# HamidGadirov/OpticalFlowSciVis

Hardware: AMD Instinct MI355X
Metric: volume-pairs/sec, Flow-3D unsupervised train step (fwd+loss+bwd+AdamW) (higher is better)
Workload: dtype f32

## Files before the change

include/flowsci_hip.h:

```cpp
#ifndef FLOWSCI_HIP_H
#define FLOWSCI_HIP_H

#ifdef __cplusplus
extern "C" {
#endif

typedef void* fs_stream_t;

enum {
  FS_OK = 0,
  FS_ERR_NULLPTR = 1,
  FS_ERR_SHAPE = 2,
  FS_ERR_ARG = 3,
  FS_ERR_LAUNCH = 4,
  FS_ERR_UNSUPPORTED = 5
};

#define FS_ABI_VERSION 380
int fs_version(void);
const char* fs_error_string(int code);

int fs_warp3d_fwd(const float* in, const float* flow, float* out,
                  int B, int C, const int* in_dhw, int D, int H, int W, fs_stream_t stream);
int fs_warp3d_bwd(const float* in, const float* flow, const float* grad_out,
                  float* grad_in, float* grad_flow,
                  int B, int C, const int* in_dhw, int D, int H, int W, fs_stream_t stream);

int fs_warp3d_pair_fwd(const float* img0, const float* img1, const float* flow6,
                       float* out0, float* out1,
                       int B, int C, const int* in_dhw, int D, int H, int W, fs_stream_t stream);
int fs_warp3d_pair_bwd(const float* img0, const float* img1, const float* flow6,
                       const float* grad_out0, const float* grad_out1,
                       float* grad_img0, float* grad_img1, float* grad_flow6,
                       int B, int C, const int* in_dhw, int D, int H, int W, fs_stream_t stream);
int fs_warp3d_pair_bwd_acc(const float* img0, const float* img1, const float* flow6,
                           const float* grad_out0, const float* grad_out1,
                           float* grad_img0, float* grad_img1,
                           const float* grad_flow_add, float* grad_flow6,
                           int B, int C, const int* in_dhw, int D, int H, int W, fs_stream_t stream);

int fs_upsample_warp3d_pair_fwd(const float* img0, const float* img1, const float* delta,
                                const float* prev_flow, float* flow_out, float* out0, float* out1,
                                int B, int C, const int* in_dhw, int Ds, int Hs, int Ws, int factor,
                                float scale, fs_stream_t stream);
int fs_upsample_warp3d_pair_bwd(const float* img0, const float* img1, const float* flow6,
                                const float* grad_out0, const float* grad_out1,
                                const float* grad_flow_add, float* grad_flow_total, float* grad_delta,
                                float* ws, int B, int C, const int* in_dhw, int Ds, int Hs, int Ws,
                                int factor, float scale, fs_stream_t stream);
int fs_warp3d_pair_bwd_acc3(const float* img0, const float* img1, const float* flow6,
                            const float* grad_out0, long long gout_batch_stride0, const float* grad_out1,
                            long long gout_batch_stride1, float* grad_img0, float* grad_img1,
                            const float* add0, long long batch_stride0, const float* add1, long long batch_stride1,
                            const float* add2, long long batch_stride2, float* grad_flow6,
                            int B, int C, const int* in_dhw, int D, int H, int W, fs_stream_t stream);
int fs_upsample_warp3d_pair_bwd3(const float* img0, const float* img1, const float* flow6,
                                 const float* grad_out0, long long gout_batch_stride0, const float* grad_out1,
                                 long long gout_batch_stride1, const float* add0, long long batch_stride0, const float* add1, long long batch_stride1,
                                 const float* add2, long long batch_stride2, float* grad_flow_total, float* grad_delta,
                                 float* ws, int B, int C, const int* in_dhw, int Ds, int Hs, int Ws,
                                 int factor, float scale, fs_stream_t stream);

enum { FS_W3_KERNEL_GATHER = 0, FS_W3_KERNEL_RC = 1 };
int fs_warp3d_kernel_id(const float* in0, const float* in1, const float* flow, int B, int C, const int* in_dhw,
                        int D, int H, int W, int backward, int with_grad_in);

enum { FS_WARP2D_RIFE = 0, FS_WARP2D_PWC = 1, FS_WARP2D_PHOTO = 2, FS_WARP2D_DILATED = 3 };

int fs_warp2d_fwd(const float* in, const float* flow, const float* start, float* out,
                  int B, int C, const int* in_hw, int H, int W, int mode, int with_mask,
                  fs_stream_t stream);
int fs_warp2d_bwd(const float* in, const float* flow, const float* start,
                  const float* grad_out, float* grad_in, float* grad_flow,
                  int B, int C, const int* in_hw, int H, int W, int mode, int with_mask,
                  fs_stream_t stream);

int fs_warp2d_pair_fwd(const float* img0, const float* img1, const float* flow4,
                       float* out0, float* out1,
// ... 265 lines not shown
```

opticalflowscivis_amd/_lib.py:

```python
import ctypes
import os

import torch

_HERE = os.path.dirname(os.path.abspath(__file__))
PRODUCT_LIB_PATH = os.path.join(_HERE, "csrc", "libflowsci_hip.so")
LIB_PATH = os.environ.get("FLOWSCI_HIP_LIBRARY") or PRODUCT_LIB_PATH
ABLATION = LIB_PATH != PRODUCT_LIB_PATH


def ablation_env(name):
    return os.environ.get(name) if ABLATION else None


def switches():
    return {"library": "ablation build: " + LIB_PATH if ABLATION else "product",
            "env": {k: v for k, v in sorted(os.environ.items()) if k.startswith("FLOWSCI_")}}

ABI_VERSION = 380

_f32p = ctypes.c_void_p
_int = ctypes.c_int
_float = ctypes.c_float
_stream = ctypes.c_void_p
_intp = ctypes.POINTER(ctypes.c_int)
_i64p = ctypes.POINTER(ctypes.c_longlong)
_i64 = ctypes.c_longlong
_ptrv = ctypes.POINTER(ctypes.c_void_p)
_double = ctypes.c_double

class FsWprepJob(ctypes.Structure):
    _fields_ = [("w", ctypes.c_void_p), ("ws", ctypes.c_void_p), ("kind", ctypes.c_int), ("total", ctypes.c_int),
                ("p", ctypes.c_int * 6)]


_jobp = ctypes.POINTER(FsWprepJob)

SIGNATURES = {
    "fs_version": [],
    "fs_error_string": [_int],
    "fs_warp3d_fwd": [_f32p] * 3 + [_int, _int, _intp, _int, _int, _int, _stream],
    "fs_warp3d_bwd": [_f32p] * 5 + [_int, _int, _intp, _int, _int, _int, _stream],
    "fs_warp3d_pair_fwd": [_f32p] * 5 + [_int, _int, _intp, _int, _int, _int, _stream],
    "fs_warp3d_pair_bwd": [_f32p] * 8 + [_int, _int, _intp, _int, _int, _int, _stream],
    "fs_warp3d_pair_bwd_acc": [_f32p] * 9 + [_int, _int, _intp, _int, _int, _int, _stream],
    "fs_warp3d_pair_bwd_acc3": [_f32p] * 3 + [_f32p, _i64, _f32p, _i64] + [_f32p] * 2 + [_f32p, _i64, _f32p, _i64, _f32p, _i64, _f32p, _int, _int, _intp, _int, _int,
                                _int, _stream],
    "fs_upsample_warp3d_pair_bwd3": [_f32p] * 3 + [_f32p, _i64, _f32p, _i64] + [_f32p, _i64, _f32p, _i64, _f32p, _i64] + [_f32p] * 3 +
                                    [_int, _int, _intp, _int, _int, _int, _int, _float, _stream],
    "fs_upsample_warp3d_pair_fwd": [_f32p] * 7 + [_int, _int, _intp, _int, _int, _int, _int, _float, _stream],
    "fs_upsample_warp3d_pair_bwd": [_f32p] * 9 + [_int, _int, _intp, _int, _int, _int, _int, _float, _stream],
    "fs_warp2d_pair_fwd": [_f32p] * 5 + [_int, _int, _intp, _int, _int, _int, _stream],
    "fs_warp2d_pair_bwd": [_f32p] * 8 + [_int, _int, _intp, _int, _int, _int, _stream],
    "fs_interp3d_bwd_scaled": [_f32p] * 3 + [_int] * 10 + [_float, _stream],
    "fs_downsample3d_fwd": [_f32p] * 2 + [_int] * 6 + [_float, _stream],
    "fs_downsample3d_fwd_ms": [_ptrv, _i64p, _f32p] + [_int] * 6 + [_float, _stream],
    "fs_resize2d_fwd": [_f32p] * 2 + [_int] * 8 + [_float, _stream],
    "fs_resize2d_bwd": [_f32p] * 2 + [_int] * 8 + [_float, _stream],
    "fs_occ_check2d": [_f32p] * 4 + [_int] * 3 + [_float, _float, _int, _stream],
    "fs_laploss2d_sizes": [_int] * 4 + [_i64p] * 3,
    "fs_laploss2d_fwd": [_f32p] * 5 + [_int] * 4 + [_stream],
    "fs_laploss2d_bwd": [_f32p] * 4 + [_int] * 4 + [_stream],
    "fs_laploss3d_sizes": [_int] * 5 + [_i64p] * 3,
    "fs_laploss3d_fwd": [_f32p] * 5 + [_int] * 5 + [_stream],
    "fs_laploss3d_bwd": [_f32p] * 4 + [_int] * 5 + [_stream],
    "fs_conv3d_fwd_ws_floats": [_int] * 3,
    "fs_conv3d_fwd": [_f32p] * 5 + [_int] * 13 + [_stream],
    "fs_upsample3d_scale_add": [_f32p] * 3 + [_int] * 6 + [_float, _stream],
    "fs_conv3d_fwd_dprelu_part_floats": [_int] * 5,
    "fs_conv3d_fwd_dprelu_part_floats_k3": [_int] * 5,
# ... 44 lines not shown
    "fs_warp2d_bwd": [_f32p, _f32p, _f32p, _f32p, _f32p, _f32p, _int, _int, _intp, _int, _int, _int, _int,
                      _stream],
    "fs_frame_metrics2d_ws_bytes": [_int] * 4,
    "fs_frame_metrics3d_ws_bytes": [_int] * 5,
    "fs_frame_metrics2d": [_f32p] * 2 + [_int] * 4 + [_double] + [_f32p] * 3 + [_stream],
    "fs_frame_metrics3d": [_f32p] * 2 + [_int] * 5 + [_double] + [_f32p] * 3 + [_stream],
    "fs_flow_metrics2d_ws_bytes": [_int] * 4,
    "fs_flow_metrics3d_ws_bytes": [_int] * 6,
    "fs_flow_metrics2d": [_f32p] * 2 + [_int] * 4 + [_i64] * 2 + [_f32p] * 2 + [_float] * 2 + [_f32p] * 3 + [_stream],
    "fs_flow_metrics3d": [_f32p] * 2 + [_int] * 5 + [_i64] * 2 + [_f32p] * 2 + [_int] + [_float] * 2 + [_f32p] * 3 +
                         [_stream],
    "fs_flow_consistency2d_ws_bytes": [_int] * 4,
    "fs_flow_consistency3d_ws_bytes": [_int] * 5,
    "fs_flow_consistency2d": [_f32p] * 2 + [_int] * 4 + [_i64] * 2 + [_f32p] * 3 + [_double] * 2 + [_f32p] * 4 + [_stream],
    "fs_flow_consistency3d": [_f32p] * 2 + [_int] * 5 + [_i64] * 2 + [_f32p] * 3 + [_double] * 2 + [_f32p] * 4 + [_stream],
    "fs_triplet_gather": [_f32p, _int, _i64, _int, _int, _int, _f32p, _int, _int, _int, _int, _f32p, _stream],
    "fs_series_stats_ws_bytes": [_int, _i64],
    "fs_series_stats": [_f32p, _int, _int, _i64, _f32p, _f32p, _stream],
    "fs_census3d_dist_fwd": [_f32p] * 3 + [_int] * 5 + [_stream],
    "fs_census3d_dist_bwd": [_f32p] * 5 + [_int] * 5 + [_stream],
    "fs_flow_smooth3d_fwd": [_f32p] * 4 + [_int] * 5 + [_float] * 3 + [_stream],
    "fs_flow_smooth3d_bwd": [_f32p] * 4 + [_int] * 5 + [_float] * 3 + [_stream],
}
_RESTYPES = {"fs_error_string": ctypes.c_char_p, "fs_conv3d_fwd_ws_floats": ctypes.c_longlong,
             "fs_conv3d_wrw_det_ws_floats": ctypes.c_longlong,
             "fs_frame_metrics2d_ws_bytes": ctypes.c_longlong, "fs_frame_metrics3d_ws_bytes": ctypes.c_longlong,
             "fs_flow_metrics2d_ws_bytes": ctypes.c_longlong, "fs_flow_metrics3d_ws_bytes": ctypes.c_longlong,
             "fs_flow_consistency2d_ws_bytes": ctypes.c_longlong, "fs_flow_consistency3d_ws_bytes": ctypes.c_longlong,
             "fs_series_stats_ws_bytes": ctypes.c_longlong,
             "fs_conv3d_tr_ws_floats": ctypes.c_longlong, "fs_conv3d_fwd_dprelu_part_floats": ctypes.c_longlong,
             "fs_conv3d_fwd_dprelu_part_floats_k3": ctypes.c_longlong}


class FlowsciLibraryError(RuntimeError):
    pass


class FlowsciKernelError(RuntimeError):
    pass


_lib = None


def lib():
    global _lib
    if _lib is not None:
# ... 29 lines not shown
```

opticalflowscivis_amd/convgrad.py:

```python
import os

import torch
import torch.nn as nn
import torch.nn.functional as F


def _tuple(v, nd):
    return tuple(v) if isinstance(v, (tuple, list)) else (v,) * nd


_stock_seen = set()


def _note_stock_path(what, x, w, stride, padding):
    if x.dim() != 5 or not x.is_cuda or x.dtype != torch.float32:
        return
    key = (what, tuple(x.shape[1:]), tuple(w.shape), tuple(stride), tuple(padding))
    if key in _stock_seen:
        return
    _stock_seen.add(key)
    import warnings
    warnings.warn("opticalflowscivis_amd: %s of a 3-D convolution runs on stock ATen / MIOpen kernels, not on the HIP "
                  "implicit-GEMM kernels (input %s, weight %s, stride %s, padding %s: unsupported geometry or beyond "
                  "32-bit offsets)" % (what, tuple(x.shape), tuple(w.shape), tuple(stride), tuple(padding)),
# ... 116 lines not shown


class _ConvTrAddFn(torch.autograd.Function):

    @staticmethod
    def forward(ctx, x, w, b, addend, stride, padding):
        from . import ops
        y = ops.conv3d_tr(x, w, b, None, None, addend)
        ctx.save_for_backward(x, w)
        ctx.cfg = (stride, padding, b is not None)
        return y

    @staticmethod
    def backward(ctx, gy):
        x, w = ctx.saved_tensors
        stride, padding, has_bias = ctx.cfg
        gy = gy.contiguous()
        gx = gw = gb = None
        if ctx.needs_input_grad[0]:
            gx = _conv_grad_input(x, w, gy, stride, padding, True)
        if ctx.needs_input_grad[1]:
            gw = _conv_grad_weight(x, w, gy, stride, padding, True)
        if has_bias and ctx.needs_input_grad[2]:
            gb = gy.sum(dim=(0, 2, 3, 4))
        return gx, gw, gb, (gy if ctx.needs_input_grad[3] else None), None, None


class _ConvPReLUFn(torch.autograd.Function):

    @staticmethod
    def forward(ctx, x, w, b, a, stride, padding, transposed):
        y, z = _conv_forward(x, w, b, stride, padding, transposed, a)
        ctx.save_for_backward(x, w, y, a)
        ctx.cfg = (stride, padding, transposed, b is not None)
        return z

    @staticmethod
    def backward(ctx, gz):
        from . import ops
        x, w, y, a = ctx.saved_tensors
        stride, padding, transposed, has_bias = ctx.cfg
        gy, ga, gb = ops.prelu_backward(y, gz.contiguous(), a, want_bias_grad=has_bias)
        gx = gw = None
        if ctx.needs_input_grad[0]:
            gx = _conv_grad_input(x, w, gy, stride, padding, transposed)
        if ctx.needs_input_grad[1]:
            gw = _conv_grad_weight(x, w, gy, stride, padding, transposed)
# ... 59 lines not shown
        return None
    return _ConvPReLUCatFn.apply(conv.weight, conv.bias, act.weight, _tuple(conv.stride, 3), _tuple(conv.padding, 3),
                                 *pieces)


class _HeadFn(torch.autograd.Function):

    @staticmethod
    def forward(ctx, x, w1, b1, a1, w2, b2, addend):
        from . import ops
        y1, z1 = ops.conv3d_tr(x, w1, b1, None, a1)
        out = ops.conv3d_tr(z1, w2, b2, None, None, addend)
        ctx.save_for_backward(x, w1, a1, y1, z1, w2)
        ctx.has = (b1 is not None, b2 is not None, addend is not None)
        return out

    @staticmethod
    def backward(ctx, gout):
        from . import ops
        x, w1, a1, y1, z1, w2 = ctx.saved_tensors
        s3, p3 = (2, 2, 2), (1, 1, 1)
        gout = gout.contiguous()
        gw2 = _conv_grad_weight(z1, w2, gout, s3, p3, True) if ctx.needs_input_grad[4] else None
        gb2 = gout.sum(dim=(0, 2, 3, 4)) if (ctx.has[1] and ctx.needs_input_grad[5]) else None
        fused = ops.conv3d_deconv_grad_input_dprelu(gout, w2, y1, a1)
        if fused is not None:
            gy1, ga1, gb1 = fused
        else:
            gz1 = _conv_grad_input(z1, w2, gout, s3, p3, True)
            gy1, ga1, gb1 = ops.prelu_backward(y1, gz1, a1, want_bias_grad=ctx.has[0])
        if not ctx.has[0]:
            gb1 = None
        gw1 = _conv_grad_weight(x, w1, gy1, s3, p3, True) if ctx.needs_input_grad[1] else None
        gx = _conv_grad_input(x, w1, gy1, s3, p3, True) if ctx.needs_input_grad[0] else None
        return gx, gw1, gb1, ga1, gw2, gb2, (gout if (ctx.has[2] and ctx.needs_input_grad[6]) else None)


def head_fused_ok(head, x, addend):
    d1, act, d2 = head[0], head[1], head[2]
    if not (_hip_autograd(x) and x.dim() == 5 and x.dtype == torch.float32 and isinstance(d1, ConvTranspose3d)
            and isinstance(d2, ConvTranspose3d) and isinstance(act, nn.PReLU)):
        return False
    for d in (d1, d2):
        if not (_tuple(d.kernel_size, 3) == (4, 4, 4) and _tuple(d.stride, 3) == (2, 2, 2) and _tuple(d.padding, 3) == (1, 1, 1)
                and d.groups == 1 and _tuple(d.dilation, 3) == (1, 1, 1) and _tuple(d.output_padding, 3) == (0, 0, 0)):
            return False
    if act.weight.numel() not in (1, d1.out_channels):
# ... 130 lines not shown
```

opticalflowscivis_amd/csrc/warp3d.hip:

```cpp
#include <stdint.h>

#include <type_traits>

#include "common.hpp"

namespace {

constexpr int TH = 64;

struct W3P {
  int B, C, D, H, W;
  int Di, Hi, Wi;
  int tilesH, tilesW;
  int dc, nDC;
  float stepD, stepH, stepW;
  float rD, rH, rW;
  float mD, mH, mW;
  unsigned rowB, planeB;
  int flowC;
};

struct W3Fwd { const float* in[2]; float* out[2]; };
struct W3Bwd {
  const float* in[2]; const float* gout[2]; float* gin[2];
  long long gbs[2];
};

// ... 725 lines not shown
  if (vec && rc_mode() != 0 && rc::applicable(p, io.in[0], io.in[1]))
    return {W3K::RC, (int)FS_AB_ENV_LL("FLOWSCI_W3_RC_DC", rc::pick_dc(p, npair))};
  return {vec ? W3K::RING_VEC : W3K::RING_SCALAR, (int)FS_AB_ENV_LL("FLOWSCI_W3_RING_DC", 16)};
}

W3Pick pick_bwd(const W3P& p, const W3Bwd& io, int npair, bool with_gin, const float* flow, const float* gflow,
                const W3Add& gadd) {
  const bool vec = vec_ok(p, flow, gflow, io.gout[0], io.gout[1]) && vec_ok(p, gadd.a[0], gadd.a[1], gadd.a[2], nullptr) &&
                   gadd.bs[0] % 4 == 0 && gadd.bs[1] % 4 == 0 && gadd.bs[2] % 4 == 0 && io.gbs[0] % 4 == 0 && io.gbs[1] % 4 == 0;
  if (vec && rc_mode() != 0 && !with_gin && gflow != nullptr && rc::applicable(p, io.in[0], io.in[1]))
    return {W3K::RC, (int)FS_AB_ENV_LL("FLOWSCI_W3_RC_DC", rc::pick_dc(p, npair))};
  return {vec ? W3K::BWD_VEC : W3K::BWD_SCALAR, p.dc};
}

dim3 set_chunks(W3P& p, const W3Pick& k, int npair) {
  p.flowC = 3 * npair;
  p.dc = k.dc;
  p.nDC = fs::cdiv(p.D, p.dc);
  return dim3((unsigned)((long long)p.B * p.nDC * p.tilesH * p.tilesW), npair);
}

template <bool BWD, int NMW_, int R>
void launch_rc(const dim3& g, hipStream_t st, const W3Fwd& fio, const W3Bwd& bio, const float* flow, float* gflow,
               const W3Add& gadd, const W3P& p) {
  const dim3 bc(64 * (NCW + NMW_));
#ifdef FS_ABLATION
#define W3_RC_DBG(N) \
  if (rc_mode() == 10 + N) { hipLaunchKernelGGL((rc::warp3d_rc_kernel<BWD, NMW_, R, N>), g, bc, 0, st, fio, bio, flow, gflow, gadd, p); return; }
  W3_RC_DBG(1) W3_RC_DBG(2) W3_RC_DBG(3)
#endif
  hipLaunchKernelGGL((rc::warp3d_rc_kernel<BWD, NMW_, R>), g, bc, 0, st, fio, bio, flow, gflow, gadd, p);
}

int launch_fwd(const W3Fwd& io, int npair, const float* flow, const UpP* up, W3P& p, fs_stream_t stream) {
  const W3Pick k = pick_fwd(p, io, npair, flow, up);
  const dim3 g = set_chunks(p, k, npair);
  hipStream_t st = (hipStream_t)stream;
  switch (k.kernel) {
    case W3K::UPS_VEC: hipLaunchKernelGGL((warp3d_fwd_kernel<512, true, true>), g, dim3(512), 0, st, io, flow, *up, p); break;
    case W3K::UPS_SCALAR: hipLaunchKernelGGL((warp3d_fwd_kernel<512, false, true>), g, dim3(512), 0, st, io, flow, *up, p); break;
    case W3K::RC: launch_rc<false, 2, 6>(g, st, io, W3Bwd{}, flow, nullptr, W3Add{}, p); break;
    case W3K::RING_VEC: {
#ifdef FS_ABLATION
      static const int ring = (int)FS_AB_ENV_LL("FLOWSCI_W3_RING", 0);
#define W3_RING_CASE(R, A, DBG, ID) \
      if (ring == ID) { hipLaunchKernelGGL((warp3d_fwd_ring_kernel<true, A, R, DBG>), g, dim3(NT2), 0, st, io, flow, p); break; }
      W3_RING_CASE(3, 0, 0, 3) W3_RING_CASE(4, 0, 0, 4) W3_RING_CASE(5, 0, 0, 5) W3_RING_CASE(3, 2, 0, 13) W3_RING_CASE(5, 2, 0, 15)
      W3_RING_CASE(4, 2, 1, 101) W3_RING_CASE(4, 2, 2, 102) W3_RING_CASE(4, 2, 3, 103) W3_RING_CASE(4, 2, 4, 104) W3_RING_CASE(4, 2, 5, 105)
#endif
      hipLaunchKernelGGL((warp3d_fwd_ring_kernel<true, 2, 4>), g, dim3(NT2), 0, st, io, flow, p);
      break;
    }
    case W3K::RING_SCALAR: hipLaunchKernelGGL((warp3d_fwd_ring_kernel<false, 0, 3>), g, dim3(NT2), 0, st, io, flow, p); break;
    default: return FS_ERR_ARG;
  }
  FS_LAUNCH_CHECK();
  return FS_OK;
}

int launch_bwd(const W3Bwd& io, int npair, bool with_gin, const float* flow, float* gflow, const W3Add& gadd,
               W3P& p, fs_stream_t stream) {
  const W3Pick k = pick_bwd(p, io, npair, with_gin, flow, gflow, gadd);
  const dim3 g = set_chunks(p, k, npair);
  hipStream_t st = (hipStream_t)stream;
  switch (k.kernel) {
    case W3K::RC: launch_rc<true, 4, 5>(g, st, W3Fwd{}, io, flow, gflow, gadd, p); break;
    case W3K::BWD_VEC:
      if (with_gin) hipLaunchKernelGGL((warp3d_bwd_kernel<256, true, true>), g, dim3(256), 0, st, io, flow, gflow, gadd, p);
      else hipLaunchKernelGGL((warp3d_bwd_kernel<256, true, false>), g, dim3(256), 0, st, io, flow, gflow, gadd, p);
      break;
    case W3K::BWD_SCALAR:
      if (with_gin) hipLaunchKernelGGL((warp3d_bwd_kernel<256, false, true>), g, dim3(256), 0, st, io, flow, gflow, gadd, p);
      else hipLaunchKernelGGL((warp3d_bwd_kernel<256, false, false>), g, dim3(256), 0, st, io, flow, gflow, gadd, p);
      break;
    default: return FS_ERR_ARG;
  }
  FS_LAUNCH_CHECK();
  return FS_OK;
}

int make_params_up(W3P& p, int B, int C, const int* in_dhw, int Ds, int Hs, int Ws, int factor) {
  if (factor != 2 && factor != 4) return FS_ERR_ARG;
  if (Ds < 1 || Hs < 1 || Ws < 1) return FS_ERR_SHAPE;
  if ((long long)Ds * Hs * Ws * factor * factor * factor >= (1ll << 31)) return FS_ERR_SHAPE;
  return make_params(p, B, C, in_dhw, Ds * factor, Hs * factor, Ws * factor);
}

}

extern "C" int fs_warp3d_fwd(const float* in, const float* flow, float* out, int B, int C,
                             const int* in_dhw, int D, int H, int W, fs_stream_t stream) {
  FS_ENTER();
  FS_REQUIRE_PTR(in); FS_REQUIRE_PTR(flow); FS_REQUIRE_PTR(out);
  W3P p;
  if (const int rc = make_params(p, B, C, in_dhw, D, H, W); rc != FS_OK) return rc;
  W3Fwd io = {{in, nullptr}, {out, nullptr}};
  return launch_fwd(io, 1, flow, nullptr, p, stream);
}
// ... 55 lines not shown

extern "C" int fs_warp3d_pair_bwd_acc3(const float* img0, const float* img1, const float* flow6,
                                       const float* grad_out0, long long gout_batch_stride0, const float* grad_out1,
                                       long long gout_batch_stride1, float* grad_img0,
                                       float* grad_img1, const float* add0, long long batch_stride0,
                                       const float* add1, long long batch_stride1, const float* add2,
                                       long long batch_stride2, float* grad_flow6, int B, int C, const int* in_dhw,
                                       int D, int H, int W, fs_stream_t stream) {
  FS_ENTER();
  FS_REQUIRE_PTR(img0); FS_REQUIRE_PTR(img1); FS_REQUIRE_PTR(flow6);
  FS_REQUIRE_PTR(grad_out0); FS_REQUIRE_PTR(grad_out1); FS_REQUIRE_PTR(grad_flow6);
  if ((grad_img0 == nullptr) != (grad_img1 == nullptr)) return FS_ERR_NULLPTR;
  W3P p;
  if (const int rc = make_params(p, B, C, in_dhw, D, H, W); rc != FS_OK) return rc;
  const long long fl = (long long)6 * D * H * W;
  if ((add0 && batch_stride0 < fl) || (add1 && batch_stride1 < fl) || (add2 && batch_stride2 < fl)) return FS_ERR_ARG;
  const long long gl = (long long)C * D * H * W;
  if ((gout_batch_stride0 && gout_batch_stride0 < gl) || (gout_batch_stride1 && gout_batch_stride1 < gl)) return FS_ERR_ARG;
  W3Bwd io = {{img0, img1}, {grad_out0, grad_out1}, {grad_img0, grad_img1}, {gout_batch_stride0, gout_batch_stride1}};
  return launch_bwd(io, 2, grad_img0 != nullptr, flow6, grad_flow6,
                    W3Add{{add0, add1, add2}, {batch_stride0, batch_stride1, batch_stride2}}, p, stream);
}

extern "C" int fs_warp3d_kernel_id(const float* in0, const float* in1, const float* flow, int B, int C, const int* in_dhw,
                                   int D, int H, int W, int backward, int with_grad_in) {
  W3P p;
  if (const int rc = make_params(p, B, C, in_dhw, D, H, W); rc != FS_OK) return -rc;
  alignas(16) float al[4];
  const int npair = in1 != nullptr ? 2 : 1;
  const W3Pick k = backward ? pick_bwd(p, W3Bwd{{in0, in1}, {al, al}, {}, {}}, npair, with_grad_in != 0, flow, al, W3Add{})
                            : pick_fwd(p, W3Fwd{{in0, in1}, {al, al}}, npair, flow, nullptr);
  return k.kernel == W3K::RC ? FS_W3_KERNEL_RC : FS_W3_KERNEL_GATHER;
}

extern "C" int fs_upsample_warp3d_pair_fwd(const float* img0, const float* img1, const float* delta,
                                           const float* prev_flow, float* flow_out, float* out0, float* out1,
                                           int B, int C, const int* in_dhw, int Ds, int Hs, int Ws, int factor,
                                           float scale, fs_stream_t stream) {
  FS_ENTER();
  FS_REQUIRE_PTR(img0); FS_REQUIRE_PTR(img1); FS_REQUIRE_PTR(delta); FS_REQUIRE_PTR(flow_out);
  FS_REQUIRE_PTR(out0); FS_REQUIRE_PTR(out1);
  W3P p;
  if (const int rc = make_params_up(p, B, C, in_dhw, Ds, Hs, Ws, factor); rc != FS_OK) return rc;
  UpP u = {delta, prev_flow, flow_out, Ds, Hs, Ws, 1.0f / (float)factor, scale};
  W3Fwd io = {{img0, img1}, {out0, out1}};
  return launch_fwd(io, 2, nullptr, &u, p, stream);
// ... 37 lines not shown
```

opticalflowscivis_amd/csrc/warp3d_rc.hpp:

```cpp
#pragma once

namespace rc {

constexpr int NP = 37;
constexpr int NQ = 18;
constexpr int NX = 4 * NQ;
constexpr int ROW_INSTR = 11;
constexpr int RSLOTS = 64 * ROW_INSTR;
constexpr unsigned PLB = NX * 4u;
constexpr unsigned RSB = RSLOTS * 16u;
constexpr int NFR = 3;

struct Mail {
  int xb, zb;
  int lo[2], nv[2], sl[2];
  int st[2][NCW][2];
};

template <bool BWD>
struct SampI {
  float ax, ay, az;
  float mx, my, mz;
  int x0, y0, z0;
  bool px, py, pz;
// ... 78 lines not shown
      voff[i] = ((unsigned)min(hq[i], p.H - 1) * (unsigned)p.W + (unsigned)min(wq[i], p.W - 4)) * 4u;
    }
  }
  __device__ __forceinline__ void dma(const float* plane, float4* tile) const {
#if defined(__HIP_DEVICE_COMPILE__)
    __amdgpu_buffer_rsrc_t r = __builtin_amdgcn_make_buffer_rsrc((void*)plane, (short)0, 0x7fffffff, 0x00020000);
#pragma unroll
    for (int i = 0; i < NJ; ++i)
      __builtin_amdgcn_raw_ptr_buffer_load_lds(r, (lds_ptr_t)(tile + 64 * (NJ * m + i)), 16, voff[i], 0, 0, 2);
#endif
  }
  __device__ __forceinline__ void get(const float4* tile, float4 (&v)[NJ]) const {
#pragma unroll
    for (int i = 0; i < NJ; ++i) v[i] = tile[64 * (NJ * m + i) + (threadIdx.x & 63)];
  }
  __device__ __forceinline__ void ldg(const float* plane, float4 (&v)[NJ]) const {
#pragma unroll
    for (int i = 0; i < NJ; ++i) v[i] = *reinterpret_cast<const float4*>(reinterpret_cast<const char*>(plane) + voff[i]);
  }
  __device__ __forceinline__ void put(float* plane, const W3P& p, const float4 (&v)[NJ]) const {
#pragma unroll
    for (int i = 0; i < NJ; ++i)
      if (hq[i] < p.H && wq[i] < p.W) *reinterpret_cast<float4*>(plane + (size_t)hq[i] * p.W + wq[i]) = v[i];
  }
};

__device__ __forceinline__ void tile_minmax(const float4* tile, float& mn, float& mx) {
  const int lane = threadIdx.x & 63;
  float a = INFINITY, b = -INFINITY;
#pragma unroll
  for (int i = 0; i < TSLOTS / 64; ++i) {
    const float4 v = tile[64 * i + lane];
    a = fminf(fminf(a, v.x), fminf(fminf(v.y, v.z), v.w));
    b = fmaxf(fmaxf(b, v.x), fmaxf(fmaxf(v.y, v.z), v.w));
  }
#pragma unroll
  for (int o = 32; o > 0; o >>= 1) {
    a = fminf(a, __shfl_xor(a, o, 64));
    b = fmaxf(b, __shfl_xor(b, o, 64));
  }
  mn = a; mx = b;
}

__device__ __forceinline__ void decode_tile_xcd(const W3P& p, int& b, int& d0, int& h0, int& w0) {
  const int nb = gridDim.x;
  int bid = blockIdx.x;
  const int per = nb >> 3;
  if ((nb & 7) == 0) bid = (bid & 7) * per + (bid >> 3);
  const int tw = bid % p.tilesW; bid /= p.tilesW;
  const int th = bid % p.tilesH; bid /= p.tilesH;
  const int dk = bid % p.nDC;
  b = bid / p.nDC;
  d0 = dk * p.dc;
  h0 = th * TH;
  w0 = tw * TW;
}

template <bool BWD, int NMW_, int R, int DBG = 0>
__global__ __launch_bounds__(64 * (NCW + NMW_)) void warp3d_rc_kernel(W3Fwd fio, W3Bwd bio, const float* __restrict__ flow,
                                                                      float* gflow, W3Add gadd, W3P p) {
  constexpr int NPL = BWD ? 4 : 3;
  __shared__ float4 sF[NFR][NPL][TSLOTS];
  __shared__ float4 sO[BWD ? 1 : 2][BWD ? 1 : TSLOTS];
  __shared__ float4 sC[R][RSLOTS];
  __shared__ Mail mail;
  using TL = TileLane<NMW_>;

  const float* __restrict__ in = BWD ? bio.in[blockIdx.y] : fio.in[blockIdx.y];
  int b, d0, h0, w0;
  decode_tile_xcd(p, b, d0, h0, w0);
  const int HW = p.H * p.W;
  const size_t vol = (size_t)p.D * HW;
  const size_t ivol = (size_t)p.Di * p.Hi * p.Wi;
  const float* fb = flow + ((size_t)b * p.flowC + 3 * blockIdx.y) * vol;
  const float* __restrict__ vin = in + (size_t)b * ivol;
  const int n = min(d0 + p.dc, p.D) - d0;
  const int lane = threadIdx.x & 63;
  const int wv = __builtin_amdgcn_readfirstlane((int)(threadIdx.x >> 6));

  if (wv >= NCW) {
    TL tl;
    tl.init(p, wv - NCW, lane, h0, w0);
    const int m = wv - NCW;
// ... 71 lines not shown
        const int nchi = max(min(chi_t, clo + R), chi);
        for (int y = chi; y < nchi; ++y) {
          int s = sclo + (y - clo);
          s -= (s >= R) ? R : 0;
          s -= (s >= R) ? R : 0;
          load_row(y, s);
        }
        chi = nchi;
        const int nclo = max(max(clo, chi - R), min(lo_req, chi));
        int s = sclo + (nclo - clo);
        s -= (s >= R) ? R : 0;
        s -= (s >= R) ? R : 0;
        sclo = s; clo = nclo;
      }
      if (m == 0 && lane == 0) {
        mail.lo[kn & 1] = clo; mail.nv[kn & 1] = ok ? chi - clo : 0; mail.sl[kn & 1] = sclo;
      }
    };
    if (m == 0 && lane == 0) { mail.xb = xb; mail.zb = zb; }
    advance(0, a0, b0 + 2);
    wait_vm(0);
    w3_lds_barrier();
    float4 ad[BWD ? 3 : 1][BWD ? 3 : 1][TL::NJ];
    for (int k = 0; k < n; ++k) {
      if (k > 0) {
        if constexpr (BWD) {
          wait_vm(k + 1 < n ? DMA_PER : 0);
          float* g = gfb + (size_t)(d0 + k - 1) * HW;
#pragma unroll
          for (int c = 0; c < 3; ++c) {
            float4 v[TL::NJ];
            tl.get(sF[(k - 1) % NFR][c], v);
#pragma unroll
            for (int a = 0; a < 3; ++a)
              if (gab[a] != nullptr) {
#pragma unroll
                for (int i = 0; i < TL::NJ; ++i) {
                  v[i].x += ad[a][c][i].x; v[i].y += ad[a][c][i].y; v[i].z += ad[a][c][i].z; v[i].w += ad[a][c][i].w;
                }
              }
            tl.put(g + (size_t)c * vol, p, v);
          }
        } else {
          float4 v[TL::NJ];
          tl.get(sO[(k - 1) & 1], v);
          tl.put(outb + (size_t)(d0 + k - 1) * HW, p, v);
        }
      }
      int younger = 0;
      if (k + 1 < n) {
        int a, bb, sh;
        if (k == 0) { a = a0; bb = b0; sh = 1; }
        else {
          int mn = mail.st[(k - 1) & 1][lane & (NCW - 1)][0], mx = mail.st[(k - 1) & 1][lane & (NCW - 1)][1];
#pragma unroll
          for (int o = 1; o < NCW; o <<= 1) { mn = min(mn, __shfl_xor(mn, o, 64)); mx = max(mx, __shfl_xor(mx, o, 64)); }
          a = __builtin_amdgcn_readfirstlane(mn); bb = __builtin_amdgcn_readfirstlane(mx); sh = 2;
        }
        const int core = bb - a + 2;
        const int below = (core + 1 <= R - 1) ? 1 : 0, above = (core + below + 1 <= R - 1) ? 1 : 0;
        advance(k + 1, a + sh - below, bb + sh + 2 + above);
      }
      if constexpr (BWD) {
#pragma unroll
// ... 8 lines not shown
        asm volatile("s_waitcnt lgkmcnt(0)" ::: "memory");
        load_slice(k + 2);
        younger += DMA_PER;
      }
      wait_vm(younger);
      w3_lds_barrier();
    }
    if constexpr (BWD) {
      wait_vm(0);
      float* g = gfb + (size_t)(d0 + n - 1) * HW;
#pragma unroll
      for (int c = 0; c < 3; ++c) {
        float4 v[TL::NJ];
        tl.get(sF[(n - 1) % NFR][c], v);
#pragma unroll
        for (int a = 0; a < 3; ++a)
          if (gab[a] != nullptr) {
#pragma unroll
            for (int i = 0; i < TL::NJ; ++i) {
              v[i].x += ad[a][c][i].x; v[i].y += ad[a][c][i].y; v[i].z += ad[a][c][i].z; v[i].w += ad[a][c][i].w;
            }
          }
        tl.put(g + (size_t)c * vol, p, v);
      }
    } else {
      float4 v[TL::NJ];
      tl.get(sO[(n - 1) & 1], v);
      tl.put(outb + (size_t)(d0 + n - 1) * HW, p, v);
    }
    return;
  }
  const int hq = h0 + lane;
  const int h = min(hq, p.H - 1);
  const float lin_h = fs::linspace_pm1(h, p.H, p.stepH);
  float lin_w[4];
#pragma unroll
  for (int i = 0; i < 4; ++i) lin_w[i] = fs::linspace_pm1(min(w0 + 4 * wv + i, p.W - 1), p.W, p.stepW);
  const int slot = t_slot(lane, wv);
  const float k0 = (p.mW * 0.5f) * p.rH, k1 = (p.mH * 0.5f) * p.rD, k2 = (p.mD * 0.5f) * p.rW;
  typedef const __attribute__((address_space(3))) char* lds_cchar_t;
  const lds_cchar_t cch = (lds_cchar_t)(&sC[0][0]);
  typedef const __attribute__((address_space(3))) float* lds_cfloat_t;
  auto lds_pair = [&](unsigned off) { Pair q; lds_cfloat_t f = (lds_cfloat_t)(cch + off); q.a = f[0]; q.b = f[1]; return q; };
  w3_lds_barrier();
  w3_lds_barrier();
  const int xb = mail.xb, zb = mail.zb;
// ... 99 lines not shown
```

opticalflowscivis_amd/ops.py:

```python
import ctypes
from fractions import Fraction

import torch

from . import _lib

WARP2D_RIFE, WARP2D_PWC, WARP2D_PHOTO, WARP2D_DILATED = 0, 1, 2, 3


def _stream(t):
    return torch.cuda.current_stream(t.device).cuda_stream


def _need_cuda_f32(name, t, ndim):
    if not isinstance(t, torch.Tensor):
        raise ValueError("%s must be a tensor" % name)
    if t.dtype != torch.float32:
        raise ValueError("%s must be float32, got %s" % (name, t.dtype))
    if t.dim() != ndim:
        raise ValueError("%s must be %d-D, got shape %s" % (name, ndim, tuple(t.shape)))
    if not t.is_cuda:
        raise ValueError("%s must live on a GPU (the HIP hot path has no CPU fallback); got %s" %
                         (name, t.device))
    return t.contiguous()
# ... 307 lines not shown
        for g in keep[4:]:
            extra = extra + g
        keep = keep[:2] + [keep[2] + extra]
        args = []
        for g in keep:
            g = g.contiguous()
            args += [g.data_ptr(), int(g.stride(0))]
    while len(args) < 6:
        args += [None, 0]
    return args, keep, nbytes


def _gout_strided(g, like):
    vol = like.shape[2] * like.shape[3] * like.shape[4]
    inner = (vol, like.shape[3] * like.shape[4], like.shape[4], 1)
    if g.is_contiguous():
        return g, 0
    if (g.dim() == 5 and tuple(g.stride()[1:]) == inner and g.stride(0) >= g.shape[1] * vol and g.stride(0) % 4 == 0
            and g.data_ptr() % 16 == 0):
        return g, int(g.stride(0))
    return g.contiguous(), 0


def _pair_backward(img0, img1, flow, g0, g1, need_img, need_flow, gflow_add=None):
    if flow.dim() == 5 and gflow_add is not None:
        (g0, s0), (g1, s1) = _gout_strided(g0, flow), _gout_strided(g1, flow)
    else:
        g0, g1, s0, s1 = g0.contiguous(), g1.contiguous(), 0, 0
    gi0 = torch.zeros_like(img0) if need_img else None
    gi1 = torch.zeros_like(img1) if need_img else None
    B, C = img0.shape[:2]
    gflow = None
    with torch.cuda.device(flow.device):
        if flow.dim() == 5:
            D, H, W = flow.shape[2:]
            nb = 8 * flow.numel() + 8 * g0.numel() * 2 + (8 * img0.numel() if need_img else 0)
            mis = (img0.data_ptr() % 16, img1.data_ptr() % 16, flow.data_ptr() % 16)
            sym, fl, fq = _kernel_accounting("warp3d_bwd", mis, B, C, *img0.shape[2:], D, H, W, int(need_img))
            if gflow_add is not None:
                adds = gflow_add if isinstance(gflow_add, (list, tuple)) else [gflow_add]
                aargs, keep, abytes = _flow_addends(adds, flow)
                gflow = torch.empty_like(flow)
                _call("fs_warp3d_pair_bwd_acc3", img0.data_ptr(), img1.data_ptr(), flow.data_ptr(),
                      g0.data_ptr(), s0, g1.data_ptr(), s1, _ptr(gi0), _ptr(gi1), *aargs, gflow.data_ptr(),
                      B, C, _in_dhw(img0, flow), D, H, W, _stream(flow), algo_bytes=nb + abytes, algo_flops=fl,
                      equiv_flops=fq, kernel=sym)
                del keep
            else:
                gflow = torch.empty_like(flow) if need_flow else None
                _call("fs_warp3d_pair_bwd", img0.data_ptr(), img1.data_ptr(), flow.data_ptr(),
                      g0.data_ptr(), g1.data_ptr(), _ptr(gi0), _ptr(gi1), _ptr(gflow), B, C,
                      _in_dhw(img0, flow), D, H, W, _stream(flow), algo_bytes=nb, algo_flops=fl, equiv_flops=fq,
                      kernel=sym)
        else:
            H, W = flow.shape[2:]
            gflow = torch.empty_like(flow) if need_flow else None
            _call("fs_warp2d_pair_bwd", img0.data_ptr(), img1.data_ptr(), flow.data_ptr(),
                  g0.data_ptr(), g1.data_ptr(), _ptr(gi0), _ptr(gi1), _ptr(gflow), B, C,
                  _in_hw(img0, flow), H, W, WARP2D_RIFE, _stream(flow),
                  algo_bytes=4 * flow.numel() * (2 if need_flow else 1) + 8 * g0.numel() * (3 if need_img else 2))
            if gflow_add is not None and gflow is not None:
                for g in (gflow_add if isinstance(gflow_add, (list, tuple)) else [gflow_add]):
                    if g is not None:
                        gflow = gflow + g
    return gi0, gi1, gflow


class _WarpPair(torch.autograd.Function):
    @staticmethod
    def forward(ctx, img0, img1, flow):
        img0, img1, flow, nd = _check_pair(img0, img1, flow)
        out0, out1 = _pair_forward(img0, img1, flow, nd)
        ctx.save_for_backward(img0, img1, flow)
        return out0, out1

    @staticmethod
# ... 2040 lines not shown
```

Before: 29.57.

## Fuse per-channel flow-gradient sums into warp3d backward for conv bias grads

The warp3d pair backward kernels now also emit per-channel partial sums of the flow gradient they write. The RC kernel accumulates them in registers as it stores; other kernels get a small chunked partial-sum pass. A finish kernel reduces the partials in double and attaches the result to the gradient tensor. Conv bias-gradient code reuses these sums instead of launching a full gy.sum reduction over the volume, saving a re-read of the gradient in exchange for extra partial-buffer allocations, launches and version-tracking bookkeeping.

```diff
diff --git a/include/flowsci_hip.h b/include/flowsci_hip.h
--- a/include/flowsci_hip.h
+++ b/include/flowsci_hip.h
@@ -16,7 +16,7 @@
   FS_ERR_UNSUPPORTED = 5
 };
 
-#define FS_ABI_VERSION 380
+#define FS_ABI_VERSION 390
 int fs_version(void);
 const char* fs_error_string(int code);
 
@@ -54,6 +54,18 @@
                             const float* add0, long long batch_stride0, const float* add1, long long batch_stride1,
                             const float* add2, long long batch_stride2, float* grad_flow6,
                             int B, int C, const int* in_dhw, int D, int H, int W, fs_stream_t stream);
+long long fs_warp3d_chan_sums_part_floats(int B, int C, const int* in_dhw, int D, int H, int W);
+int fs_warp3d_pair_bwd_sums(const float* img0, const float* img1, const float* flow6,
+                            const float* grad_out0, const float* grad_out1, float* grad_img0, float* grad_img1,
+                            float* grad_flow6, float* part, long long part_floats, float* chan_sums,
+                            int B, int C, const int* in_dhw, int D, int H, int W, fs_stream_t stream);
+int fs_warp3d_pair_bwd_acc3_sums(const float* img0, const float* img1, const float* flow6,
+                                 const float* grad_out0, long long gout_batch_stride0, const float* grad_out1,
+                                 long long gout_batch_stride1, float* grad_img0, float* grad_img1,
+                                 const float* add0, long long batch_stride0, const float* add1, long long batch_stride1,
+                                 const float* add2, long long batch_stride2, float* grad_flow6,
+                                 float* part, long long part_floats, float* chan_sums,
+                                 int B, int C, const int* in_dhw, int D, int H, int W, fs_stream_t stream);
 int fs_upsample_warp3d_pair_bwd3(const float* img0, const float* img1, const float* flow6,
                                  const float* grad_out0, long long gout_batch_stride0, const float* grad_out1,
                                  long long gout_batch_stride1, const float* add0, long long batch_stride0, const float* add1, long long batch_stride1,
diff --git a/opticalflowscivis_amd/_lib.py b/opticalflowscivis_amd/_lib.py
--- a/opticalflowscivis_amd/_lib.py
+++ b/opticalflowscivis_amd/_lib.py
@@ -17,7 +17,7 @@
     return {"library": "ablation build: " + LIB_PATH if ABLATION else "product",
             "env": {k: v for k, v in sorted(os.environ.items()) if k.startswith("FLOWSCI_")}}
 
-ABI_VERSION = 380
+ABI_VERSION = 390
 
 _f32p = ctypes.c_void_p
 _int = ctypes.c_int
@@ -46,6 +46,11 @@
     "fs_warp3d_pair_bwd_acc": [_f32p] * 9 + [_int, _int, _intp, _int, _int, _int, _stream],
     "fs_warp3d_pair_bwd_acc3": [_f32p] * 3 + [_f32p, _i64, _f32p, _i64] + [_f32p] * 2 + [_f32p, _i64, _f32p, _i64, _f32p, _i64, _f32p, _int, _int, _intp, _int, _int,
                                 _int, _stream],
+    "fs_warp3d_chan_sums_part_floats": [_int, _int, _intp, _int, _int, _int],
+    "fs_warp3d_pair_bwd_sums": [_f32p] * 8 + [_f32p, _i64, _f32p] + [_int, _int, _intp, _int, _int, _int, _stream],
+    "fs_warp3d_pair_bwd_acc3_sums": [_f32p] * 3 + [_f32p, _i64, _f32p, _i64] + [_f32p] * 2 +
+                                    [_f32p, _i64, _f32p, _i64, _f32p, _i64, _f32p] + [_f32p, _i64, _f32p] +
+                                    [_int, _int, _intp, _int, _int, _int, _stream],
     "fs_upsample_warp3d_pair_bwd3": [_f32p] * 3 + [_f32p, _i64, _f32p, _i64] + [_f32p, _i64, _f32p, _i64, _f32p, _i64] + [_f32p] * 3 +
                                     [_int, _int, _intp, _int, _int, _int, _int, _float, _stream],
     "fs_upsample_warp3d_pair_fwd": [_f32p] * 7 + [_int, _int, _intp, _int, _int, _int, _int, _float, _stream],
@@ -136,7 +141,8 @@
     "fs_flow_smooth3d_fwd": [_f32p] * 4 + [_int] * 5 + [_float] * 3 + [_stream],
     "fs_flow_smooth3d_bwd": [_f32p] * 4 + [_int] * 5 + [_float] * 3 + [_stream],
 }
-_RESTYPES = {"fs_error_string": ctypes.c_char_p, "fs_conv3d_fwd_ws_floats": ctypes.c_longlong,
+_RESTYPES = {"fs_error_string": ctypes.c_char_p, "fs_warp3d_chan_sums_part_floats": ctypes.c_longlong,
+             "fs_conv3d_fwd_ws_floats": ctypes.c_longlong,
              "fs_conv3d_wrw_det_ws_floats": ctypes.c_longlong,
              "fs_frame_metrics2d_ws_bytes": ctypes.c_longlong, "fs_frame_metrics3d_ws_bytes": ctypes.c_longlong,
              "fs_flow_metrics2d_ws_bytes": ctypes.c_longlong, "fs_flow_metrics3d_ws_bytes": ctypes.c_longlong,
diff --git a/opticalflowscivis_amd/convgrad.py b/opticalflowscivis_amd/convgrad.py
--- a/opticalflowscivis_amd/convgrad.py
+++ b/opticalflowscivis_amd/convgrad.py
@@ -162,7 +162,8 @@
         if ctx.needs_input_grad[1]:
             gw = _conv_grad_weight(x, w, gy, stride, padding, True)
         if has_bias and ctx.needs_input_grad[2]:
-            gb = gy.sum(dim=(0, 2, 3, 4))
+            from . import ops
+            gb = ops.chan_sums_or_reduce(gy)
         return gx, gw, gb, (gy if ctx.needs_input_grad[3] else None), None, None
 
 
@@ -268,7 +269,7 @@
         s3, p3 = (2, 2, 2), (1, 1, 1)
         gout = gout.contiguous()
         gw2 = _conv_grad_weight(z1, w2, gout, s3, p3, True) if ctx.needs_input_grad[4] else None
-        gb2 = gout.sum(dim=(0, 2, 3, 4)) if (ctx.has[1] and ctx.needs_input_grad[5]) else None
+        gb2 = ops.chan_sums_or_reduce(gout) if (ctx.has[1] and ctx.needs_input_grad[5]) else None
         fused = ops.conv3d_deconv_grad_input_dprelu(gout, w2, y1, a1)
         if fused is not None:
             gy1, ga1, gb1 = fused
diff --git a/opticalflowscivis_amd/csrc/chansums.hip b/opticalflowscivis_amd/csrc/chansums.hip
--- /dev/null
+++ b/opticalflowscivis_amd/csrc/chansums.hip
@@ -0,0 +1,48 @@
+#include "common.hpp"
+#include "chansums.hpp"
+
+namespace {
+
+__global__ __launch_bounds__(256) void chan_sums_finish_kernel(const float* __restrict__ part, int rows, int C,
+                                                               float* __restrict__ sums) {
+  __shared__ double red[256];
+  double s = 0.0;
+  for (int i = threadIdx.x; i < rows; i += 256) s += (double)part[(size_t)i * C + blockIdx.x];
+  red[threadIdx.x] = s;
+  __syncthreads();
+  for (int st = 128; st > 0; st >>= 1) {
+    if ((int)threadIdx.x < st) red[threadIdx.x] += red[threadIdx.x + st];
+    __syncthreads();
+  }
+  if (threadIdx.x == 0) sums[blockIdx.x] = (float)red[0];
+}
+
+__global__ __launch_bounds__(256) void chan_part_kernel(const float* __restrict__ g, int C, long long vol, int nchunk,
+                                                        float* __restrict__ part) {
+  const int b = blockIdx.y / C, c = blockIdx.y - b * C;
+  const float* src = g + (size_t)blockIdx.y * vol;
+  const long long lo = (long long)blockIdx.x * fs::kChanSumsChunk;
+  const long long hi = lo + fs::kChanSumsChunk < vol ? lo + fs::kChanSumsChunk : vol;
+  float s = 0.f;
+  for (long long i = lo + threadIdx.x; i < hi; i += 256) s += src[i];
+  __shared__ float red[4];
+  s = fs::wave_sum(s);
+  if ((threadIdx.x & 63) == 0) red[threadIdx.x >> 6] = s;
+  __syncthreads();
+  if (threadIdx.x == 0) part[((size_t)b * nchunk + blockIdx.x) * C + c] = (red[0] + red[1]) + (red[2] + red[3]);
+}
+
+}
+
+namespace fs {
+
+void launch_chan_part(const float* g, int B, int C, long long vol, float* part, hipStream_t st) {
+  const int nchunk = cdiv(vol, kChanSumsChunk);
+  hipLaunchKernelGGL(chan_part_kernel, dim3((unsigned)nchunk, (unsigned)(B * C)), dim3(256), 0, st, g, C, vol, nchunk, part);
+}
+
+void launch_chan_sums_finish(const float* part, int rows, int C, float* sums, hipStream_t st) {
+  hipLaunchKernelGGL(chan_sums_finish_kernel, dim3(C), dim3(256), 0, st, part, rows, C, sums);
+}
+
+}
diff --git a/opticalflowscivis_amd/csrc/chansums.hpp b/opticalflowscivis_amd/csrc/chansums.hpp
--- /dev/null
+++ b/opticalflowscivis_amd/csrc/chansums.hpp
@@ -0,0 +1,12 @@
+#pragma once
+#include <hip/hip_runtime.h>
+
+namespace fs {
+
+constexpr int kChanSumsChunk = 8192;
+
+void launch_chan_part(const float* g, int B, int C, long long vol, float* part, hipStream_t st);
+
+void launch_chan_sums_finish(const float* part, int rows, int C, float* sums, hipStream_t st);
+
+}
diff --git a/opticalflowscivis_amd/csrc/warp3d.hip b/opticalflowscivis_amd/csrc/warp3d.hip
--- a/opticalflowscivis_amd/csrc/warp3d.hip
+++ b/opticalflowscivis_amd/csrc/warp3d.hip
@@ -3,6 +3,7 @@
 #include <type_traits>
 
 #include "common.hpp"
+#include "chansums.hpp"
 
 namespace {
 
@@ -774,14 +775,14 @@
 
 template <bool BWD, int NMW_, int R>
 void launch_rc(const dim3& g, hipStream_t st, const W3Fwd& fio, const W3Bwd& bio, const float* flow, float* gflow,
-               const W3Add& gadd, const W3P& p) {
+               const W3Add& gadd, const W3P& p, float* part = nullptr) {
   const dim3 bc(64 * (NCW + NMW_));
 #ifdef FS_ABLATION
 #define W3_RC_DBG(N) \
-  if (rc_mode() == 10 + N) { hipLaunchKernelGGL((rc::warp3d_rc_kernel<BWD, NMW_, R, N>), g, bc, 0, st, fio, bio, flow, gflow, gadd, p); return; }
+  if (rc_mode() == 10 + N) { hipLaunchKernelGGL((rc::warp3d_rc_kernel<BWD, NMW_, R, N>), g, bc, 0, st, fio, bio, flow, gflow, gadd, p, part); return; }
   W3_RC_DBG(1) W3_RC_DBG(2) W3_RC_DBG(3)
 #endif
-  hipLaunchKernelGGL((rc::warp3d_rc_kernel<BWD, NMW_, R>), g, bc, 0, st, fio, bio, flow, gflow, gadd, p);
+  hipLaunchKernelGGL((rc::warp3d_rc_kernel<BWD, NMW_, R>), g, bc, 0, st, fio, bio, flow, gflow, gadd, p, part);
 }
 
 int launch_fwd(const W3Fwd& io, int npair, const float* flow, const UpP* up, W3P& p, fs_stream_t stream) {
@@ -810,13 +811,30 @@
   return FS_OK;
 }
 
+constexpr int RC_BWD_NMW = 4;
+constexpr int CS_CHUNK = fs::kChanSumsChunk;
+
+long long cs_rows_rc(const W3P& p, int npair) {
+  const int dc = (int)FS_AB_ENV_LL("FLOWSCI_W3_RC_DC", rc::pick_dc(p, npair));
+  return (long long)p.B * fs::cdiv(p.D, dc > 0 ? dc : 1) * p.tilesH * p.tilesW * RC_BWD_NMW;
+}
+long long cs_rows_pass(const W3P& p) { return (long long)p.B * fs::cdiv((long long)p.D * p.H * p.W, CS_CHUNK); }
+
 int launch_bwd(const W3Bwd& io, int npair, bool with_gin, const float* flow, float* gflow, const W3Add& gadd,
-               W3P& p, fs_stream_t stream) {
+               W3P& p, fs_stream_t stream, float* part = nullptr, long long part_floats = 0, float* sums = nullptr) {
+  if (sums != nullptr && (part == nullptr || gflow == nullptr)) return FS_ERR_NULLPTR;
   const W3Pick k = pick_bwd(p, io, npair, with_gin, flow, gflow, gadd);
   const dim3 g = set_chunks(p, k, npair);
   hipStream_t st = (hipStream_t)stream;
+  const int fc = 3 * npair;
+  long long rows = 0;
+  if (sums != nullptr) {
+    rows = k.kernel == W3K::RC ? (long long)g.x * RC_BWD_NMW : cs_rows_pass(p);
+    if (rows * fc > part_floats || rows >= (1ll << 31)) return FS_ERR_ARG;
+    if (k.kernel != W3K::RC && (long long)p.B * fc > 65535) return FS_ERR_SHAPE;
+  }
   switch (k.kernel) {
-    case W3K::RC: launch_rc<true, 4, 5>(g, st, W3Fwd{}, io, flow, gflow, gadd, p); break;
+    case W3K::RC: launch_rc<true, RC_BWD_NMW, 5>(g, st, W3Fwd{}, io, flow, gflow, gadd, p, sums ? part : nullptr); break;
     case W3K::BWD_VEC:
       if (with_gin) hipLaunchKernelGGL((warp3d_bwd_kernel<256, true, true>), g, dim3(256), 0, st, io, flow, gflow, gadd, p);
       else hipLaunchKernelGGL((warp3d_bwd_kernel<256, true, false>), g, dim3(256), 0, st, io, flow, gflow, gadd, p);
@@ -826,6 +844,12 @@
       else hipLaunchKernelGGL((warp3d_bwd_kernel<256, false, false>), g, dim3(256), 0, st, io, flow, gflow, gadd, p);
       break;
     default: return FS_ERR_ARG;
+  }
+  if (sums != nullptr) {
+    if (k.kernel != W3K::RC) {
+      fs::launch_chan_part(gflow, p.B, fc, (long long)p.D * p.H * p.W, part, st);
+    }
+    fs::launch_chan_sums_finish(part, (int)rows, fc, sums, st);
   }
   FS_LAUNCH_CHECK();
   return FS_OK;
@@ -927,6 +951,53 @@
                     W3Add{{add0, add1, add2}, {batch_stride0, batch_stride1, batch_stride2}}, p, stream);
 }
 
+extern "C" long long fs_warp3d_chan_sums_part_floats(int B, int C, const int* in_dhw, int D, int H, int W) {
+  W3P p;
+  if (make_params(p, B, C, in_dhw, D, H, W) != FS_OK) return 0;
+  const long long a = cs_rows_rc(p, 2), b = cs_rows_pass(p);
+  return 6 * (a > b ? a : b);
+}
+
+extern "C" int fs_warp3d_pair_bwd_sums(const float* img0, const float* img1, const float* flow6,
+                                       const float* grad_out0, const float* grad_out1, float* grad_img0,
+                                       float* grad_img1, float* grad_flow6, float* part, long long part_floats,
+                                       float* chan_sums, int B, int C, const int* in_dhw, int D, int H, int W,
+                                       fs_stream_t stream) {
+  FS_ENTER();
+  FS_REQUIRE_PTR(img0); FS_REQUIRE_PTR(img1); FS_REQUIRE_PTR(flow6);
+  FS_REQUIRE_PTR(grad_out0); FS_REQUIRE_PTR(grad_out1); FS_REQUIRE_PTR(grad_flow6);
+  FS_REQUIRE_PTR(part); FS_REQUIRE_PTR(chan_sums);
+  if ((grad_img0 == nullptr) != (grad_img1 == nullptr)) return FS_ERR_NULLPTR;
+  W3P p;
+  if (const int rc = make_params(p, B, C, in_dhw, D, H, W); rc != FS_OK) return rc;
+  W3Bwd io = {{img0, img1}, {grad_out0, grad_out1}, {grad_img0, grad_img1}};
+  return launch_bwd(io, 2, grad_img0 != nullptr, flow6, grad_flow6, W3Add{}, p, stream, part, part_floats, chan_sums);
+}
+
+extern "C" int fs_warp3d_pair_bwd_acc3_sums(const float* img0, const float* img1, const float* flow6,
+                                            const float* grad_out0, long long gout_batch_stride0, const float* grad_out1,
+                                            long long gout_batch_stride1, float* grad_img0, float* grad_img1,
+                                            const float* add0, long long batch_stride0, const float* add1,
+                                            long long batch_stride1, const float* add2, long long batch_stride2,
+                                            float* grad_flow6, float* part, long long part_floats, float* chan_sums,
+                                            int B, int C, const int* in_dhw, int D, int H, int W, fs_stream_t stream) {
+  FS_ENTER();
+  FS_REQUIRE_PTR(img0); FS_REQUIRE_PTR(img1); FS_REQUIRE_PTR(flow6);
+  FS_REQUIRE_PTR(grad_out0); FS_REQUIRE_PTR(grad_out1); FS_REQUIRE_PTR(grad_flow6);
+  FS_REQUIRE_PTR(part); FS_REQUIRE_PTR(chan_sums);
+  if ((grad_img0 == nullptr) != (grad_img1 == nullptr)) return FS_ERR_NULLPTR;
+  W3P p;
+  if (const int rc = make_params(p, B, C, in_dhw, D, H, W); rc != FS_OK) return rc;
+  const long long fl = (long long)6 * D * H * W;
+  if ((add0 && batch_stride0 < fl) || (add1 && batch_stride1 < fl) || (add2 && batch_stride2 < fl)) return FS_ERR_ARG;
+  const long long gl = (long long)C * D * H * W;
+  if ((gout_batch_stride0 && gout_batch_stride0 < gl) || (gout_batch_stride1 && gout_batch_stride1 < gl)) return FS_ERR_ARG;
+  W3Bwd io = {{img0, img1}, {grad_out0, grad_out1}, {grad_img0, grad_img1}, {gout_batch_stride0, gout_batch_stride1}};
+  return launch_bwd(io, 2, grad_img0 != nullptr, flow6, grad_flow6,
+                    W3Add{{add0, add1, add2}, {batch_stride0, batch_stride1, batch_stride2}}, p, stream, part, part_floats,
+                    chan_sums);
+}
+
 extern "C" int fs_warp3d_kernel_id(const float* in0, const float* in1, const float* flow, int B, int C, const int* in_dhw,
                                    int D, int H, int W, int backward, int with_grad_in) {
   W3P p;
diff --git a/opticalflowscivis_amd/csrc/warp3d_rc.hpp b/opticalflowscivis_amd/csrc/warp3d_rc.hpp
--- a/opticalflowscivis_amd/csrc/warp3d_rc.hpp
+++ b/opticalflowscivis_amd/csrc/warp3d_rc.hpp
@@ -124,6 +124,13 @@
 #pragma unroll
     for (int i = 0; i < NJ; ++i)
       if (hq[i] < p.H && wq[i] < p.W) *reinterpret_cast<float4*>(plane + (size_t)hq[i] * p.W + wq[i]) = v[i];
+  }
+  __device__ __forceinline__ float stored_sum(const W3P& p, const float4 (&v)[NJ]) const {
+    float s = 0.f;
+#pragma unroll
+    for (int i = 0; i < NJ; ++i)
+      if (hq[i] < p.H && wq[i] < p.W) s += (v[i].x + v[i].y) + (v[i].z + v[i].w);
+    return s;
   }
 };
 
@@ -160,7 +167,7 @@
 
 template <bool BWD, int NMW_, int R, int DBG = 0>
 __global__ __launch_bounds__(64 * (NCW + NMW_)) void warp3d_rc_kernel(W3Fwd fio, W3Bwd bio, const float* __restrict__ flow,
-                                                                      float* gflow, W3Add gadd, W3P p) {
+                                                                      float* gflow, W3Add gadd, W3P p, float* part) {
   constexpr int NPL = BWD ? 4 : 3;
   __shared__ float4 sF[NFR][NPL][TSLOTS];
   __shared__ float4 sO[BWD ? 1 : 2][BWD ? 1 : TSLOTS];
@@ -278,6 +285,7 @@
     wait_vm(0);
     w3_lds_barrier();
     float4 ad[BWD ? 3 : 1][BWD ? 3 : 1][TL::NJ];
+    float cs[3] = {0.f, 0.f, 0.f};
     for (int k = 0; k < n; ++k) {
       if (k > 0) {
         if constexpr (BWD) {
@@ -296,6 +304,7 @@
                 }
               }
             tl.put(g + (size_t)c * vol, p, v);
+            if (part != nullptr) cs[c] += tl.stored_sum(p, v);
           }
         } else {
           float4 v[TL::NJ];
@@ -350,6 +359,14 @@
             }
           }
         tl.put(g + (size_t)c * vol, p, v);
+        if (part != nullptr) cs[c] += tl.stored_sum(p, v);
+      }
+      if (part != nullptr) {
+#pragma unroll
+        for (int c = 0; c < 3; ++c) {
+          const float s = fs::wave_sum(cs[c]);
+          if (lane == 0) part[((size_t)blockIdx.x * NMW_ + m) * p.flowC + 3 * blockIdx.y + c] = s;
+        }
       }
     } else {
       float4 v[TL::NJ];
diff --git a/opticalflowscivis_amd/ops.py b/opticalflowscivis_amd/ops.py
--- a/opticalflowscivis_amd/ops.py
+++ b/opticalflowscivis_amd/ops.py
@@ -353,6 +353,26 @@
     return g.contiguous(), 0
 
 
+_CHAN_SUMS = _lib.ablation_env("FLOWSCI_CHAN_SUMS") != "0"
+
+
+def _attach_chan_sums(grad, sums):
+    grad._fs_chan_sums = (sums, grad._version)
+    return grad
+
+
+def chan_sums_of(grad):
+    got = getattr(grad, "_fs_chan_sums", None)
+    if got is None or got[1] != grad._version or got[0].shape[0] != grad.shape[1]:
+        return None
+    return got[0]
+
+
+def chan_sums_or_reduce(grad):
+    s = chan_sums_of(grad)
+    return s if s is not None else grad.sum(dim=(0, 2, 3, 4))
+
+
 def _pair_backward(img0, img1, flow, g0, g1, need_img, need_flow, gflow_add=None):
     if flow.dim() == 5 and gflow_add is not None:
         (g0, s0), (g1, s1) = _gout_strided(g0, flow), _gout_strided(g1, flow)
@@ -368,21 +388,41 @@
             nb = 8 * flow.numel() + 8 * g0.numel() * 2 + (8 * img0.numel() if need_img else 0)
             mis = (img0.data_ptr() % 16, img1.data_ptr() % 16, flow.data_ptr() % 16)
             sym, fl, fq = _kernel_accounting("warp3d_bwd", mis, B, C, *img0.shape[2:], D, H, W, int(need_img))
+            sums = part = None
+            if _CHAN_SUMS and (gflow_add is not None or need_flow):
+                nf = int(_lib.lib().fs_warp3d_chan_sums_part_floats(B, C, _in_dhw(img0, flow), D, H, W))
+                if nf > 0:
+                    part, sums = flow.new_empty(nf), flow.new_empty(6)
             if gflow_add is not None:
                 adds = gflow_add if isinstance(gflow_add, (list, tuple)) else [gflow_add]
                 aargs, keep, abytes = _flow_addends(adds, flow)
                 gflow = torch.empty_like(flow)
-                _call("fs_warp3d_pair_bwd_acc3", img0.data_ptr(), img1.data_ptr(), flow.data_ptr(),
-                      g0.data_ptr(), s0, g1.data_ptr(), s1, _ptr(gi0), _ptr(gi1), *aargs, gflow.data_ptr(),
-                      B, C, _in_dhw(img0, flow), D, H, W, _stream(flow), algo_bytes=nb + abytes, algo_flops=fl,
-                      equiv_flops=fq, kernel=sym)
+                if sums is not None:
+                    _call("fs_warp3d_pair_bwd_acc3_sums", img0.data_ptr(), img1.data_ptr(), flow.data_ptr(),
+                          g0.data_ptr(), s0, g1.data_ptr(), s1, _ptr(gi0), _ptr(gi1), *aargs, gflow.data_ptr(),
+                          part.data_ptr(), part.numel(), sums.data_ptr(),
+                          B, C, _in_dhw(img0, flow), D, H, W, _stream(flow), algo_bytes=nb + abytes, algo_flops=fl,
+                          equiv_flops=fq, kernel=sym, record_as="fs_warp3d_pair_bwd_acc3")
+                else:
+                    _call("fs_warp3d_pair_bwd_acc3", img0.data_ptr(), img1.data_ptr(), flow.data_ptr(),
+                          g0.data_ptr(), s0, g1.data_ptr(), s1, _ptr(gi0), _ptr(gi1), *aargs, gflow.data_ptr(),
+                          B, C, _in_dhw(img0, flow), D, H, W, _stream(flow), algo_bytes=nb + abytes, algo_flops=fl,
+                          equiv_flops=fq, kernel=sym)
                 del keep
             else:
                 gflow = torch.empty_like(flow) if need_flow else None
-                _call("fs_warp3d_pair_bwd", img0.data_ptr(), img1.data_ptr(), flow.data_ptr(),
-                      g0.data_ptr(), g1.data_ptr(), _ptr(gi0), _ptr(gi1), _ptr(gflow), B, C,
-                      _in_dhw(img0, flow), D, H, W, _stream(flow), algo_bytes=nb, algo_flops=fl, equiv_flops=fq,
-                      kernel=sym)
+                if sums is not None:
+                    _call("fs_warp3d_pair_bwd_sums", img0.data_ptr(), img1.data_ptr(), flow.data_ptr(),
+                          g0.data_ptr(), g1.data_ptr(), _ptr(gi0), _ptr(gi1), gflow.data_ptr(), part.data_ptr(),
+                          part.numel(), sums.data_ptr(), B, C, _in_dhw(img0, flow), D, H, W, _stream(flow),
+                          algo_bytes=nb, algo_flops=fl, equiv_flops=fq, kernel=sym, record_as="fs_warp3d_pair_bwd")
+                else:
+                    _call("fs_warp3d_pair_bwd", img0.data_ptr(), img1.data_ptr(), flow.data_ptr(),
+                          g0.data_ptr(), g1.data_ptr(), _ptr(gi0), _ptr(gi1), _ptr(gflow), B, C,
+                          _in_dhw(img0, flow), D, H, W, _stream(flow), algo_bytes=nb, algo_flops=fl, equiv_flops=fq,
+                          kernel=sym)
+            if sums is not None:
+                _attach_chan_sums(gflow, sums)
         else:
             H, W = flow.shape[2:]
             gflow = torch.empty_like(flow) if need_flow else None
```

New measurement: 29.74 (median of 6 runs). No clear change (+0.6%).
